# aa217/Neural-Speech-Decoding

Measured on AMD Instinct MI355X. Metric: EEG-trials/sec (train fwd+bwd), higher is better.
Workload: dtype f32; 1 GPU; cfg2: 3-class EEG_LSTM train step (dropout 0.6 + RReLU noise, CE, Adam), 8ch x 250-step windows, H=48 L=2 fp32, batch 256/GPU; batch_per_gpu=256, global_batch=256, T=250, C=8, H=48, L=2, K=3, bidirectional=False, weights=reference checkpoint, parallelism=dp1, launch=eager

## Files before the change

neural-speech-decoding_amd/csrc/nsd_lstm2_bwd48.hip:

```cpp
#include "nsd_args.h"
#include "nsd_multi.h"
#include "nsd_prof.h"
#include "nsd_ring_block.h"
#include "nsd_bf16.h"
#include <type_traits>
#include <utility>

namespace {

constexpr int H = 48;
constexpr int G4 = 192;
constexpr int dl0(const int nb) { return nb == 1 ? 3 : 0; }
constexpr int PRIO1_CHAIN = 2, PRIO1_X1 = 3, PRIO2_CHAIN = 3, PRIO2_X1 = 2, PRIO_LOADER = 1;
constexpr int RING = 8;
constexpr int NTHREADS = 1024;
#ifndef NSD_DW_SLEEP
#define NSD_DW_SLEEP 0
#endif
#ifndef NSD_LD_SLEEP
#define NSD_LD_SLEEP 0
#endif
constexpr int DW_SLEEP = NSD_DW_SLEEP, LD_SLEEP = NSD_LD_SLEEP;
constexpr int CHUNK = 8;
constexpr int REC = 288;
// ... 8 lines not shown
    unsigned short wa[2][2][2][WK][ARS];
    unsigned short wb[2][2][2][WK][BRS];
    float pf[2][2][H][8];
    float din1x[8][H];
};
struct NoWin {};
template <int NB>
struct Smem {
    float ring[2][RING][NB][G4];
    float din1[2][NB][H];
    float stage[2][NB][2][CHUNK][REC];
    float xst[2][NB][CHUNK][8];
    typename std::conditional<NB == 1, DwWin, NoWin>::type win;
};

typedef float f32x2 __attribute__((ext_vector_type(2)));
__device__ __forceinline__ f32x2 pk_fma(f32x2 a, f32x2 b, f32x2 c) { return __builtin_elementwise_fma(a, b, c); }

__device__ __forceinline__ float slice_dot_t(const float *dv, const f32x2 (&wp)[4][6]) {
    f32x2 acc[4];
#pragma unroll
    for (int q = 0; q < 3; ++q) {
        const float4 v = *reinterpret_cast<const float4 *>(dv + 4 * q);
        const f32x2 lo = {v.x, v.y}, hi = {v.z, v.w};
#pragma unroll
        for (int jj = 0; jj < 4; ++jj) {
            acc[jj] = q == 0 ? wp[jj][0] * lo : pk_fma(wp[jj][2 * q], lo, acc[jj]);
            acc[jj] = pk_fma(wp[jj][2 * q + 1], hi, acc[jj]);
        }
    }
    const int lane = threadIdx.x;
    const bool odd = (lane & 1) != 0, hi2 = (lane & 2) != 0;
    const float r0 = acc[0].x + acc[0].y, r1 = acc[1].x + acc[1].y;
    const float r2 = acc[2].x + acc[2].y, r3 = acc[3].x + acc[3].y;
    const float ra = (odd ? r1 : r0) + quad_xor1(odd ? r0 : r1);
    const float rb = (odd ? r3 : r2) + quad_xor1(odd ? r2 : r3);
    float v = (hi2 ? rb : ra) + quad_xor2(hi2 ? ra : rb);
    v += row_ror<4>(v);
    v += row_ror<8>(v);
    return v;
}

__device__ __forceinline__ void load_wT(const float *w, const int og, const int kk, f32x2 (&wp)[4][6]) {
#pragma unroll
    for (int jj = 0; jj < 4; ++jj)
#pragma unroll
        for (int p = 0; p < 6; ++p) {
            wp[jj][p].x = w[(size_t)(12 * kk + 2 * p) * H + 4 * og + jj];
            wp[jj][p].y = w[(size_t)(12 * kk + 2 * p + 1) * H + 4 * og + jj];
        }
}

struct PrepIn { float4 gc; float cprev, ct, mk; float2 ad; };
__device__ __forceinline__ PrepIn prep_load(const Lstm2BwdArgs &a, Smem<1> &sm, const int mn, const int layer, const int u, const float cT1) {
    const int T = a.T;
    const int t = layer == 1 ? T - 1 - mn : T + 1 + dl0(1) - mn;
    const float *rec = &sm.stage[(mn >> 3) & 1][0][layer][mn & 7][0];
    const float *recp = &sm.stage[((mn - 1) >> 3) & 1][0][layer][(mn - 1) & 7][0];
    PrepIn in;
    in.gc = *reinterpret_cast<const float4 *>(rec + 4 * u);
    in.cprev = t > 0 ? rec[192 + u] : 0.f;
    in.ct = t == T - 1 ? cT1 : recp[192 + u];
    in.ad = make_float2(0.f, 0.f); in.mk = 1.f;
    if (layer == 1) in.ad = *reinterpret_cast<const float2 *>(rec + 240);
    else if (a.mask || a.rng.on) in.mk = rec[240 + u];
    return in;
}
__device__ __forceinline__ void prep_finish(Smem<1> &sm, const PrepIn &in, const int mn, const int layer, const int u, const float dpu, const float awu) {
    const float ig = in.gc.x, fg = in.gc.y, gg = in.gc.z, og = in.gc.w;
    const float tc = fast_tanh(in.ct);
    const float x = layer == 1 ? fmaf(in.ad.x, dpu, in.ad.y * awu) : in.mk;
    float *o = &sm.win.pf[mn & 1][layer][u][0];
    *reinterpret_cast<float4 *>(o) = make_float4(og * (1.f - tc * tc), fg, x, 0.f);
    *reinterpret_cast<float4 *>(o + 4) = make_float4(gg * (ig * (1.f - ig)), in.cprev * (fg * (1.f - fg)), ig * (1.f - gg * gg), tc * (og * (1.f - og)));
}
__device__ __forceinline__ void prep_layer(const Lstm2BwdArgs &a, Smem<1> &sm, const int mn, const int layer, const int u,
                                           const float dpu, const float awu, const float cT1) {
    const PrepIn in = prep_load(a, sm, mn, layer, u, cT1);
    prep_finish(sm, in, mn, layer, u, dpu, awu);
}

template <int NB, class A>
__device__ __forceinline__ void chain_role(const A &a, Smem<NB> &sm, const int layer, const int r,
                                           const int n_steps) {
    const int og = r >> 4, kk = r & 15;
    const int j = 4 * og + (r & 3), s = (r >> 2) & 3;
    const int T = a.T, B = a.B;
    const float *cseq = layer == 0 ? a.cseq0 : a.cseq1;
    f32x2 wp[4][6];
    load_wT(layer == 0 ? a.w_hh0 : a.w_hh1, og, kk, wp);
    const float awj = a.attn_w[j];
    float db = 0.f;
    Prof prof = prof_init(a.dbg);

    const int ngrp = (B + NB - 1) / NB;
    for (int grp = wg_id(a); grp < ngrp; grp += wg_count(a)) {
        const int b0 = grp * NB;
        float dc[NB], dhrec[NB], ct[NB], dpj[NB];
#pragma unroll
        for (int n = 0; n < NB; ++n) {
            const int b = b0 + n;
            dc[n] = 0.f; dhrec[n] = 0.f;
            dpj[n] = (NB == 2 && layer == 1 && b < B) ? a.dpooled[(size_t)b * H + j] : 0.f;
            ct[n] = (NB == 2 && b < B) ? cseq[((size_t)b * T + (T - 1)) * H + j] : 0.f;
        }
        step_barrier<false>(prof);

        const int tb = layer == 1 ? T - 1 : T + 1 + dl0(NB);
        for (int m0 = 0; m0 < n_steps; m0 += CHUNK) {
            const int sb = (m0 / CHUNK) & 1;
            ring_block<NB, CHUNK>(m0 >= tb - T + 2 && m0 + CHUNK - 1 <= tb, [&](const int k, const auto inside) {
                const int t = tb - (m0 + k);
                const bool active = inside.value || (t >= 0 && t < T);
                const bool prev_active = inside.value || (t + 1 >= 0 && t + 1 < T);
                if constexpr (NB == 1) {
                    const float *pfl = &sm.win.pf[k & 1][layer][j][0];
                    const float4 pf = *reinterpret_cast<const float4 *>(pfl);
                    const float qr = pfl[4 + s];
                    const float dout = layer == 1 ? pf.z : sm.win.din1x[(k + 6 - dl0(NB)) & 7][j] * pf.z;
                    if (prev_active) dhrec[0] = slice_dot_t(&sm.ring[layer][(k + RING - 1) & (RING - 1)][0][12 * kk], wp);
                    if (active) {
                        const float dht = dout + dhrec[0];
                        const float dct = fmaf(dht, pf.x, dc[0]);
                        const float mine = (s == 3 ? dht : dct) * qr;
                        dc[0] = dct * pf.y;
                        db += mine;
                        sm.ring[layer][k][0][s * H + j] = mine;
                    }
                } else
#pragma unroll
                for (int n = 0; n < NB; ++n) {
                    const float *rec = &sm.stage[sb][n][layer][k][0];
                    const float4 gc = *reinterpret_cast<const float4 *>(rec + 4 * j);
                    const float own = rec[4 * j + s];
                    const float cprev = t > 0 ? rec[192 + j] : 0.f;
                    const float aux0 = layer == 1 ? rec[240] : ((a.mask || a.rng.on) ? rec[240 + j] : 1.f);
                    const float aux1 = rec[241];
                    const float ig = gc.x, fg = gc.y, gg = gc.z, og = gc.w;
                    const float tc = fast_tanh(ct[n]);
                    const float wq = og * (1.f - tc * tc);
                    const float dact = s == 2 ? 1.f - own * own : own * (1.f - own);
                    const float qsel = s == 0 ? gg : s == 1 ? cprev : s == 2 ? ig : tc;
                    const float qr = qsel * dact;
                    float dout;
                    if (layer == 1) dout = fmaf(aux0, dpj[n], aux1 * awj);
                    else            dout = sm.din1[(k + 1) & 1][n][j] * aux0;
                    if (prev_active) dhrec[n] = slice_dot_t(&sm.ring[layer][(k + RING - 1) & (RING - 1)][n][12 * kk], wp);
                    if (active) {
                        float mine = 0.f;
                        if (b0 + n < B) {
                            const float dht = dout + dhrec[n];
                            const float dct = fmaf(dht, wq, dc[n]);
                            mine = (s == 3 ? dht : dct) * qr;
                            dc[n] = dct * fg;
                            db += mine;
                            ct[n] = cprev;
                        }
                        sm.ring[layer][k][n][s * H + j] = mine;
                    }
                }
                step_barrier<false>(prof);
            });
        }
    }
// ... 29 lines not shown
        step_barrier<false>(prof);

        for (int m0 = 0; m0 < n_steps; m0 += CHUNK) {
            const int sb = (m0 / CHUNK) & 1;
#pragma unroll
            for (int k = 0; k < CHUNK; ++k) {
                const int m = m0 + k;
                const int t1p = T - m;
                const int t0p = T + 2 - m;
                constexpr int PREV = RING - 1;
                const int e = (k + PREV) & (RING - 1);
#pragma unroll
                for (int n = 0; n < NB; ++n) {
                    const float2 xv = *reinterpret_cast<const float2 *>(&sm.xst[sb][n][k][2 * s]);
                    if (t1p >= 0 && t1p < T) {
                        float inp = slice_dot_t(&sm.ring[1][e][n][12 * kk], wp);
                        if (a.residual && b0 + n < B) {
                            const float *recp = &sm.stage[k == 0 ? sb ^ 1 : sb][n][1][e][0];
                            inp += fmaf(recp[240], dpj[n], recp[241] * awj);
                        }
                        if (s == 0) sm.din1[k & 1][n][j] = inp;
                    }
                    if (t0p >= 0 && t0p < T && b0 + n < B) {
#pragma unroll
                        for (int g = 0; g < 4; ++g) {
                            const float d = sm.ring[0][e][n][g * H + j];
                            dWih0[g][0] = fmaf(d, xv.x, dWih0[g][0]);
                            dWih0[g][1] = fmaf(d, xv.y, dWih0[g][1]);
                        }
                    }
                }
                step_barrier<false>(prof);
            }
        }
    }
    prof_store(a.dbg, prof);
    float *slab = a.slabs + (size_t)wg_id(a) * a.slab_stride;
#pragma unroll
    for (int g = 0; g < 4; ++g) {
        if (c0 < C) slab[a.o_w_ih0 + (size_t)(g * H + j) * C + c0] = dWih0[g][0];
        if (c1 < C) slab[a.o_w_ih0 + (size_t)(g * H + j) * C + c1] = dWih0[g][1];
    }
}

typedef unsigned u32x2v __attribute__((ext_vector_type(2)));
__device__ __forceinline__ float rows_reduce_scatter4(const f32x4 v) {
    const u32x2v p02 = __builtin_amdgcn_permlane32_swap(__float_as_uint(v[0]), __float_as_uint(v[2]), false, false);
    const u32x2v p13 = __builtin_amdgcn_permlane32_swap(__float_as_uint(v[1]), __float_as_uint(v[3]), false, false);
    const float s02 = __uint_as_float(p02[0]) + __uint_as_float(p02[1]);
    const float s13 = __uint_as_float(p13[0]) + __uint_as_float(p13[1]);
    const u32x2v q = __builtin_amdgcn_permlane16_swap(__float_as_uint(s02), __float_as_uint(s13), false, false);
    return __uint_as_float(q[0]) + __uint_as_float(q[1]);
}
template <class A>
__device__ __forceinline__ void x1m_role(const A &a, Smem<1> &sm, const int g, const int lane, const int n_steps) {
    const int T = a.T, B = a.B;
    const int ks = lane >> 4, ub = (lane >> 2) & 3, jc = lane & 3;
    float wv[H];
#pragma unroll
    for (int sidx = 0; sidx < H; ++sidx) wv[sidx] = a.w_ih1[(size_t)(48 * ks + sidx) * H + 16 * g + 4 * ub + jc];
    const int uo = 16 * g + 4 * ub + ks;
    const float awo = a.attn_w[uo];
    const int pu = lane < H ? lane : lane - 16, pl = g == 0 ? 1 : 0;
    const float p_aw = a.attn_w[pu];
    Prof prof = prof_init(a.dbg);
    for (int grp = wg_id(a); grp < B; grp += wg_count(a)) {
        const int b0 = grp;
        const float dpo = a.residual ? a.dpooled[(size_t)b0 * H + uo] : 0.f;
        float p_dp = 0.f, p_c = 0.f;
        if (g < 2) {
            p_dp = a.dpooled[(size_t)b0 * H + pu];
            p_c = (pl == 1 ? a.cseq1 : a.cseq0)[((size_t)b0 * T + (T - 1)) * H + pu];
        }
#pragma unroll
        for (int s4 = 0; s4 < H; s4 += 8)
            asm volatile("" : "+v"(wv[s4]), "+v"(wv[s4 + 1]), "+v"(wv[s4 + 2]), "+v"(wv[s4 + 3]), "+v"(wv[s4 + 4]), "+v"(wv[s4 + 5]), "+v"(wv[s4 + 6]), "+v"(wv[s4 + 7]));
        step_barrier<false>(prof);
        for (int m0 = 0; m0 < n_steps; m0 += CHUNK) {
#pragma unroll
            for (int k = 0; k < CHUNK; ++k) {
                const int m = m0 + k;
                PrepIn pin;
                if (g < 2) pin = prep_load(a, sm, m + 1, pl, pu, p_c);
                if ((k & 3) == 0 && m >= 4) {
                    const float *vj = &sm.ring[1][(k + 4 + jc) & 7][0][48 * ks];
                    f32x4 acc0 = {0.f, 0.f, 0.f, 0.f}, acc1 = acc0, acc2 = acc0, acc3 = acc0;
#pragma unroll
                    for (int qb = 0; qb < 12; qb += 4) {
                        f32x4 bq[4];
#pragma unroll
                        for (int q = 0; q < 4; ++q) bq[q] = *reinterpret_cast<const f32x4 *>(vj + 4 * (qb + q));
#pragma unroll
                        for (int q = 0; q < 4; ++q) {
                            acc0 = __builtin_amdgcn_mfma_f32_4x4x1f32(wv[4 * (qb + q) + 0], bq[q][0], acc0, 0, 0, 0);
                            acc1 = __builtin_amdgcn_mfma_f32_4x4x1f32(wv[4 * (qb + q) + 1], bq[q][1], acc1, 0, 0, 0);
                            acc2 = __builtin_amdgcn_mfma_f32_4x4x1f32(wv[4 * (qb + q) + 2], bq[q][2], acc2, 0, 0, 0);
                            acc3 = __builtin_amdgcn_mfma_f32_4x4x1f32(wv[4 * (qb + q) + 3], bq[q][3], acc3, 0, 0, 0);
                        }
                    }
                    float inp = rows_reduce_scatter4((acc0 + acc1) + (acc2 + acc3));
                    const int c = m - 4 + jc;
                    if (a.residual) {
                        const float *recp = &sm.stage[(c >> 3) & 1][0][1][c & 7][0];
                        inp += fmaf(recp[240], dpo, recp[241] * awo);
                    }
                    sm.win.din1x[(k + 4 + jc) & 7][uo] = inp;
                }
                if (g < 2) prep_finish(sm, pin, m + 1, pl, pu, p_dp, p_aw);
                if (g == 2 && a.da0_out && m >= 1) {
                    const int t0 = T + 2 + dl0(1) - m;
                    if (t0 >= 0 && t0 < T && lane < H)
                        *reinterpret_cast<f32x4 *>(a.da0_out + ((size_t)b0 * T + t0) * G4 + 4 * lane) =
                            *reinterpret_cast<const f32x4 *>(&sm.ring[0][(k + 7) & 7][0][4 * lane]);
                }
                step_barrier<false>(prof);
            }
        }
    }
    prof_store(a.dbg, prof);
}

template <int NB>
struct DwState {
    f32x4 acc[3][2][3];
    float bq[3][NB][3];
};

template <int Q, int NB>
__device__ __forceinline__ void dw_prefetch(const Lstm2BwdArgs &a, DwState<NB> &st, const int G, const int b0,
                                            const int lane) {
    const int T = a.T, B = a.B;
    const int i = lane & 15, k = lane >> 4;
    const int mm = 4 * G + k;
    const int t = (Q == 2) ? (T + 1 - mm) : (T - 1 - mm);
    const int tt = (Q == 1) ? t : t - 1;
    const bool ok = (t >= 0 && t < T && tt >= 0);
    const float *src = Q == 0 ? a.hseq1 : Q == 1 ? a.in1seq : a.hseq0;
#pragma unroll
    for (int n = 0; n < NB; ++n) {
        const int b = b0 + n;
#pragma unroll
        for (int nt = 0; nt < 3; ++nt)
            st.bq[Q][n][nt] = (ok && b < B) ? src[((size_t)b * T + tt) * H + 16 * nt + i] : 0.f;
    }
}

template <int Q, int NB>
__device__ __forceinline__ void dw_compute(const Lstm2BwdArgs &a, Smem<NB> &sm, DwState<NB> &st, const int G,
                                           const int dwid, const int lane) {
    const int T = a.T;
    const int i = lane & 15, k = lane >> 4;
    const int mm = 4 * G + k;
    constexpr int layer = (Q == 2) ? 0 : 1;
    const int t = layer == 1 ? (T - 1 - mm) : (T + 1 - mm);
    const bool ok = (t >= 0 && t < T);
#pragma unroll
    for (int n = 0; n < NB; ++n) {
        float av[2];
#pragma unroll
        for (int mt = 0; mt < 2; ++mt) {
            const float v = sm.ring[layer][mm & (RING - 1)][n][32 * dwid + 16 * mt + i];
            av[mt] = ok ? v : 0.f;
        }
#pragma unroll
        for (int mt = 0; mt < 2; ++mt)
#pragma unroll
            for (int nt = 0; nt < 3; ++nt)
                st.acc[Q][mt][nt] = __builtin_amdgcn_mfma_f32_16x16x4f32(av[mt], st.bq[Q][n][nt], st.acc[Q][mt][nt], 0, 0, 0);
    }
}

template <class A>
// ... 34 lines not shown
            dw_prefetch<1, NB>(a, st, G, b0, lane);
            step_barrier<false, DW_SLEEP>(prof);
            if (G > 0 && !ablated(a.ablate, 1)) dw_compute<2, NB>(a, sm, st, G - 1, dwid, lane);
            dw_prefetch<2, NB>(a, st, G, b0, lane);
            step_barrier<false, DW_SLEEP>(prof);
            step_barrier<false, DW_SLEEP>(prof);
        }
        if (!ablated(a.ablate, 1)) {
            dw_compute<0, NB>(a, sm, st, n_groups - 1, dwid, lane);
            dw_compute<1, NB>(a, sm, st, n_groups - 1, dwid, lane);
            dw_compute<2, NB>(a, sm, st, n_groups - 1, dwid, lane);
        }
    }
    prof_store(a.dbg, prof);
    float *slab = a.slabs + (size_t)wg_id(a) * a.slab_stride;
    const long base[3] = {a.o_w_hh1, a.o_w_ih1, a.o_w_hh0};
#pragma unroll
    for (int q = 0; q < 3; ++q)
#pragma unroll
        for (int mt = 0; mt < 2; ++mt)
#pragma unroll
            for (int nt = 0; nt < 3; ++nt)
#pragma unroll
                for (int rr = 0; rr < 4; ++rr) {
                    const int row = 32 * dwid + 16 * mt + 4 * (lane >> 4) + rr;
                    const int col = 16 * nt + (lane & 15);
                    slab[base[q] + (size_t)row * H + col] = st.acc[q][mt][nt][rr];
                }
}

template <class F, int... I>
__device__ __forceinline__ void static_for(F &&f, std::integer_sequence<int, I...>) { (f(std::integral_constant<int, I>{}), ...); }
__device__ __forceinline__ void split1_bf16(const float v, unsigned short &hi, unsigned short &lo) {
    const unsigned h = pack_bf16x2(v, 0.f);
    hi = (unsigned short)h;
    lo = (unsigned short)pack_bf16x2(v - bf16_lo(h), 0.f);
}
template <int RS>
__device__ __forceinline__ bf16x8 window_frag(const unsigned short *win, const int c0, const int lane) {
    const int G = lane >> 4, i = lane & 15;
    const unsigned short *p = win + (8 * (G >> 1) + (i >> 2)) * RS + c0 + 16 * (G & 1) + 4 * (i & 3);
    const s16x4 e0 = lds_read_tr16(reinterpret_cast<const bf16_t *>(p));
    const s16x4 e1 = lds_read_tr16(reinterpret_cast<const bf16_t *>(p + 4 * RS));
    return cat_tr(e0, e1);
}

__device__ __forceinline__ void split4_bf16(const f32x4 v, u32x2 &hi, u32x2 &lo) {
    hi[0] = pack_bf16x2(v[0], v[1]);
    hi[1] = pack_bf16x2(v[2], v[3]);
    lo[0] = pack_bf16x2(v[0] - bf16_lo(hi[0]), v[1] - bf16_hi(hi[0]));
    lo[1] = pack_bf16x2(v[2] - bf16_lo(hi[1]), v[3] - bf16_hi(hi[1]));
}

template <class A>
__device__ __forceinline__ void dw16_role(const A &a_in, Smem<1> &sm, const int w_in, const int lane, const int n_steps_in) {
    const int w = __builtin_amdgcn_readfirstlane(w_in), n_steps = __builtin_amdgcn_readfirstlane(n_steps_in);
    const A a = uniform_copy(a_in);
    DwWin &win = sm.win;
    const int T = a.T, B = a.B, C = a.C;
    Prof prof = prof_init(a.dbg);
    f32x16 acc[5];
#pragma unroll
    for (int q = 0; q < 5; ++q) acc[q] = zero16();
    const int l48 = lane < 48 ? lane : lane - 16;
    const float *src = w == 0 ? a.hseq1 : w == 1 ? a.in1seq : w == 2 ? a.hseq0 : a.x;
    const int rw = w == 3 ? C : H;
    const int rs = w == 3 ? lane >> 4 : l48 / 12, rp = w == 3 ? lane & 15 : l48 - 12 * rs;
    const int rl = w < 2 ? 1 : 0;
    const int rc = w == 3 ? H + rp : (w == 1 ? H : 0) + 4 * rp;
    const long sbytes = (long)B * T * rw * 4;
    const __amdgpu_buffer_rsrc_t r_s = __builtin_amdgcn_make_buffer_rsrc(const_cast<float *>(src), 0, (int)(sbytes > 0x7fffffffL ? 0x7fffffffL : sbytes), 0x00020000);
    constexpr unsigned DROP = 0x80000000u;
    const int L = w * 64 + lane, mk_k = L / H, mk_j = L - mk_k * H;
    auto gen_mask = [&](const int chunk, const int b) {
        const int t = T + 1 + dl0(1) - (chunk * CHUNK + mk_k);
        if (t >= 0 && t < T)
            sm.stage[chunk & 1][0][0][mk_k][240 + mk_j] =
                nsd_rand_u32(a.rng.seed, a.rng.base, ((uint64_t)b * T + t) * H + mk_j) < a.rng.thr_lstm ? 0.f : a.rng.keep_lstm;
    };
    bf16x8 ah, al;
    auto a_frags = [&](const int W, const int layer) {
        ah = window_frag<ARS>(&win.wa[layer][0][W & 1][0][0], 32 * w, lane);
        al = window_frag<ARS>(&win.wa[layer][1][W & 1][0][0], 32 * w, lane);
    };
    auto tile = [&](const int W, auto qc) {
        constexpr int q = decltype(qc)::value;
        constexpr int layer = q < 3 ? 1 : 0, ni = q < 3 ? q : q - 3;
        if (q == 0 || q == 3) a_frags(W, layer);
        const bf16x8 bh = window_frag<BRS>(&win.wb[layer][0][W & 1][0][0], 32 * ni, lane);
        const bf16x8 bl = window_frag<BRS>(&win.wb[layer][1][W & 1][0][0], 32 * ni, lane);
        if (!ablated(a.ablate, 1)) {
            acc[q] = __builtin_amdgcn_mfma_f32_32x32x16_bf16(ah, bh, acc[q], 0, 0, 0);
            acc[q] = __builtin_amdgcn_mfma_f32_32x32x16_bf16(al, bh, acc[q], 0, 0, 0);
            acc[q] = __builtin_amdgcn_mfma_f32_32x32x16_bf16(ah, bl, acc[q], 0, 0, 0);
        }
    };
    {
        u32x4 *z = reinterpret_cast<u32x4 *>(&win.wb[0][0][0][0][0]);
        constexpr int NZ = (int)(sizeof(win.wb) / 16);
        const u32x4 zero = {0u, 0u, 0u, 0u};
        for (int e = w * 64 + lane; e < NZ; e += 6 * 64) z[e] = zero;
    }
    const int ngrp = B;
    for (int grp = wg_id(a); grp < ngrp; grp += wg_count(a)) {
        const int b = grp;
        if (a.rng.on) gen_mask(0, b);
        auto request = [&](const int m) -> f32x4 {
            const int t = (rl == 1 ? T - 1 : T + 1 + dl0(1)) - m - rs;
            const int tt = (w == 1 || w == 3) ? t : t - 1;
            const bool ok = t >= 0 && t < T && tt >= 0 && (w != 3 || rp < C);
            f32x4 v = {0.f, 0.f, 0.f, 0.f};
            if (w == 3) {
                const unsigned off = ok ? (unsigned)((((size_t)b * T + tt) * C + rp) * 4) : DROP;
                v[0] = __uint_as_float(__builtin_amdgcn_raw_buffer_load_b32(r_s, (int)off, 0, 0));
            } else {
                const unsigned off = ok ? (unsigned)((((size_t)b * T + tt) * H + 4 * rp) * 4) : DROP;
                v = __builtin_bit_cast(f32x4, __builtin_amdgcn_raw_buffer_load_b128(r_s, (int)off, 0, 0));
            }
            return v;
        };
        f32x4 bq = {0.f, 0.f, 0.f, 0.f};
        if (w < 4) bq = request(0);
        step_barrier<false>(prof);
        auto half = [&](const int m0, auto phc) {
            constexpr int PH = decltype(phc)::value;
            static_for([&](auto kc) {
                constexpr int k = decltype(kc)::value;
                const int m = m0 + k;
                constexpr int p = PH + k;
                const int wi = (m >> 4) & 1;
                if (w >= 4 && m >= 1) {
                    const int mm = m - 1, cl = 5 - w;
                    const int t = cl == 1 ? T - 1 - mm : T + 1 + dl0(1) - mm;
                    f32x4 v = *reinterpret_cast<const f32x4 *>(&sm.ring[cl][mm & (RING - 1)][0][4 * l48]);
                    if (!(t >= 0 && t < T)) v = f32x4{0.f, 0.f, 0.f, 0.f};
                    u32x2 hi, lo;
                    split4_bf16(v, hi, lo);
                    *reinterpret_cast<u32x2 *>(&win.wa[cl][0][(mm >> 4) & 1][mm & 15][4 * l48]) = hi;
                    *reinterpret_cast<u32x2 *>(&win.wa[cl][1][(mm >> 4) & 1][mm & 15][4 * l48]) = lo;
                }
                if (w < 4 && (k & 3) == 0) {
                    if (w == 3) {
                        unsigned short hi, lo;
                        split1_bf16(bq[0], hi, lo);
                        win.wb[0][0][wi][p + rs][rc] = hi;
                        win.wb[0][1][wi][p + rs][rc] = lo;
                    } else {
                        u32x2 hi, lo;
                        split4_bf16(bq, hi, lo);
                        *reinterpret_cast<u32x2 *>(&win.wb[rl][0][wi][p + rs][rc]) = hi;
                        *reinterpret_cast<u32x2 *>(&win.wb[rl][1][wi][p + rs][rc]) = lo;
                    }
                    __builtin_amdgcn_sched_barrier(0);
                    bq = request(m + 4);
                }
                if (a.rng.on && k == 1) gen_mask((m >> 3) + 1, b);
                if (p >= 1 && p <= 5 && m >= 17) tile((m - 17) >> 4, std::integral_constant<int, (p >= 1 && p <= 5) ? p - 1 : 0>{});
                step_barrier<false, DW_SLEEP>(prof);
            }, std::make_integer_sequence<int, 8>{});
        };
        for (int m0 = 0; m0 < n_steps; m0 += 16) {
            half(m0, std::integral_constant<int, 0>{});
            if (m0 + 8 < n_steps) half(m0 + 8, std::integral_constant<int, 8>{});
        }
        {
            const int Wl = (n_steps - 1) >> 4, cl = lane >> 5, cc = 32 * w + (lane & 31);
            const int k0 = (n_steps - 1) & 15;
            for (int k = k0; k < 16; ++k) {
                win.wa[cl][0][Wl & 1][k][cc] = 0;
                win.wa[cl][1][Wl & 1][k][cc] = 0;
            }
            tile(Wl, std::integral_constant<int, 0>{});
            tile(Wl, std::integral_constant<int, 1>{});
            tile(Wl, std::integral_constant<int, 2>{});
            tile(Wl, std::integral_constant<int, 3>{});
            tile(Wl, std::integral_constant<int, 4>{});
        }
    }
    prof_store(a.dbg, prof);
    float *slab = a.slabs + (size_t)wg_id(a) * a.slab_stride;
#pragma unroll
    for (int q = 0; q < 5; ++q) {
        const int layer = q < 3 ? 1 : 0, c = 32 * (q < 3 ? q : q - 3) + (lane & 31);
        const long base = layer == 1 ? (c < H ? a.o_w_hh1 : a.o_w_ih1) : (c < H ? a.o_w_hh0 : a.o_w_ih0);
        const int ld = (layer == 0 && c >= H) ? C : H, col = c < H ? c : c - H;
        const bool okc = layer == 1 || c < H + C;
#pragma unroll
        for (int r = 0; r < 16; ++r) {
            const int row = 32 * w + mfma32_row(r, lane);
            if (okc) slab[base + (size_t)row * ld + col] = acc[q][r];
        }
    }
}

constexpr int NQ = STAGE_F4 / 64;

struct LdDesc {
    const char *base;
    int row_bytes;
    int t0;
};

template <int NB>
__device__ __forceinline__ void loader_decode(const Lstm2BwdArgs &a, const int lane, LdDesc (&d)[NQ]) {
    const int T = a.T;
#pragma unroll
    for (int q = 0; q < NQ; ++q) {
        const int e = q * 64 + lane;
        const int layer = e / (CHUNK * REC4);
        const int rem = e - layer * (CHUNK * REC4);
        const int k = rem / REC4, w = rem - k * REC4;
        d[q].t0 = layer == 1 ? (T - 1 - k) : (T + 1 + dl0(NB) - k);
        d[q].row_bytes = 0;
        d[q].base = nullptr;
        if (w < 48) {
            d[q].base = (const char *)((layer == 0 ? a.gact0 : a.gact1) + w * 4); d[q].row_bytes = H * 16;
        } else if (w < 60) {
            d[q].base = (const char *)((layer == 0 ? a.cseq0 : a.cseq1) + (w - 48) * 4) - H * 4; d[q].row_bytes = H * 4;
        } else if (layer == 0) {
            if (a.mask && !a.rng.on) { d[q].base = (const char *)(a.mask + (w - 60) * 4); d[q].row_bytes = H * 4; }
        } else if (w == 60) {
            d[q].base = (const char *)a.dsc_pack; d[q].row_bytes = 16;
        }
    }
}

template <int NB, int Q0, int Q1>
__device__ __forceinline__ void loader_issue(const Lstm2BwdArgs &a, Smem<NB> &sm, const LdDesc (&d)[NQ], const int chunk,
                                             const int buf, const int b0) {
    const int T = a.T;
#pragma unroll
    for (int n = 0; n < NB; ++n) {
        const int b = b0 + n;
        if (b < a.B) {
#pragma unroll
            for (int q = Q0; q < Q1; ++q) {
                const int t = d[q].t0 - CHUNK * chunk;
                if (d[q].row_bytes != 0 && (unsigned)t < (unsigned)T) {
                    const char *src = d[q].base + (size_t)((unsigned)(b * T + t)) * (unsigned)d[q].row_bytes;
                    __builtin_amdgcn_global_load_lds((const void *)src,
                                                     (__attribute__((address_space(3))) void *)(&sm.stage[buf][n][0][0][0] + q * 256),
                                                     16, 0, 0);
                }
            }
        }
// ... 34 lines not shown
        loader_issue<NB, 0, NQ>(a, sm, d, 0, 0, b0);
        if (NB == 2) loader_issue_x<NB>(a, sm, 0, 0, b0, lane);
        asm volatile("s_waitcnt vmcnt(0)" ::: "memory");
        if constexpr (NB == 1) { prep_layer(a, sm, 0, 1, u, dpu, awu, cT1[1]); prep_layer(a, sm, 0, 0, u, dpu, awu, cT1[0]); }
        step_barrier<true>(prof);
        for (int m0 = 0; m0 < n_steps; m0 += CHUNK) {
            const int chunk = m0 / CHUNK, nb = (chunk + 1) & 1;
            const bool on = !ablated(a.ablate, 16);
            if constexpr (NB == 1) {
                if (on) loader_issue<NB, 0, 4>(a, sm, d, chunk + 1, nb, b0);
                step_barrier<true, LD_SLEEP>(prof);
                if (on) loader_issue<NB, 4, 8>(a, sm, d, chunk + 1, nb, b0);
                step_barrier<true, LD_SLEEP>(prof);
                if (on) loader_issue<NB, 8, 12>(a, sm, d, chunk + 1, nb, b0);
                step_barrier<true, LD_SLEEP>(prof);
                if (on) loader_issue<NB, 12, 16>(a, sm, d, chunk + 1, nb, b0);
                step_barrier<true, LD_SLEEP>(prof);
                if (on) loader_issue<NB, 16, 18>(a, sm, d, chunk + 1, nb, b0);
                step_barrier<true, LD_SLEEP>(prof);
                step_barrier<true, LD_SLEEP>(prof);
                asm volatile("s_waitcnt vmcnt(0)" ::: "memory");
                step_barrier<true, LD_SLEEP>(prof);
                step_barrier<true, LD_SLEEP>(prof);
            } else {
            if (on) { loader_issue<NB, 0, 3>(a, sm, d, chunk + 1, nb, b0); if (NB == 2) loader_issue_x<NB>(a, sm, chunk + 1, nb, b0, lane); }
            step_barrier<true, LD_SLEEP>(prof);
            if (on) loader_issue<NB, 3, 6>(a, sm, d, chunk + 1, nb, b0);
            step_barrier<true, LD_SLEEP>(prof);
            if (on) loader_issue<NB, 6, 9>(a, sm, d, chunk + 1, nb, b0);
            step_barrier<true, LD_SLEEP>(prof);
            if (on) loader_issue<NB, 9, 12>(a, sm, d, chunk + 1, nb, b0);
            step_barrier<true, LD_SLEEP>(prof);
            if (on) loader_issue<NB, 12, 15>(a, sm, d, chunk + 1, nb, b0);
            step_barrier<true, LD_SLEEP>(prof);
            if (on) loader_issue<NB, 15, 18>(a, sm, d, chunk + 1, nb, b0);
            step_barrier<true, LD_SLEEP>(prof);
            step_barrier<true, LD_SLEEP>(prof);
            asm volatile("s_waitcnt vmcnt(0)" ::: "memory");
            step_barrier<true, LD_SLEEP>(prof);
            }
        }
    }
    prof_store(a.dbg, prof);
}

#define NSD_B48_ROLE_TABLE(VIEW) \
    if constexpr (NB == 1) { \
        constexpr int ROLE[16] = {0, 0, 0, 1, 1, 1, 2, 2, 2, 3, 3, 3, 3, 3, 3, 4}; \
        constexpr int PART[16] = {0, 1, 2, 0, 1, 2, 0, 1, 2, 4, 2, 3, 0, 1, 5, 0}; \
        const int lane = tid & 63; \
        const int role = ROLE[wave], part = PART[wave]; \
        if (role == 0)      { VIEW; __builtin_amdgcn_s_setprio(PRIO1_CHAIN); chain_role<NB>(a, sm, 1, 64 * part + lane, n_steps); } \
        else if (role == 1) { VIEW; __builtin_amdgcn_s_setprio(PRIO1_CHAIN); chain_role<NB>(a, sm, 0, 64 * part + lane, n_steps); } \
        else if (role == 2) { VIEW; __builtin_amdgcn_s_setprio(PRIO1_X1); x1m_role(a, sm, part, lane, n_steps); } \
        else if (role == 3) { VIEW; dw16_role(a, sm, part, lane, n_steps); } \
        else                { VIEW; __builtin_amdgcn_s_setprio(PRIO_LOADER); loader_role<NB>(a, sm, lane, n_steps); } \
    } else { \
        if (wave < 3)       { VIEW; __builtin_amdgcn_s_setprio(PRIO2_CHAIN); chain_role<NB>(a, sm, 1, tid, n_steps); } \
        else if (wave < 6)  { VIEW; __builtin_amdgcn_s_setprio(PRIO2_CHAIN); chain_role<NB>(a, sm, 0, tid - 192, n_steps); } \
        else if (wave < 9)  { VIEW; __builtin_amdgcn_s_setprio(PRIO2_X1); x1_role(a, sm, tid - 384, n_steps); } \
        else if (wave < 15) { VIEW; dw_role(a, sm, wave - 9, tid & 63, n_groups); } \
        else                { VIEW; __builtin_amdgcn_s_setprio(PRIO_LOADER); loader_role<NB>(a, sm, tid & 63, n_steps); } \
    }

#if !NSD_MULTI_TU
template <int NB>
__global__ __launch_bounds__(NTHREADS) void lstm2_bwd48_kernel(Lstm2BwdArgs a) {
    __shared__ __align__(16) Smem<NB> sm;
    const int tid = threadIdx.x;
    const int wave = __builtin_amdgcn_readfirstlane(tid >> 6);
    const int n_groups = (((a.T + 2 + dl0(NB)) / 4 + 1) + 1) & ~1;
    const int n_steps = 4 * n_groups;
    NSD_B48_ROLE_TABLE()
}

#else
template <int NB>
__global__ __launch_bounds__(NTHREADS) void lstm2_bwd48_multi_kernel(Lstm2BwdArgs a_in, ModelSplit s) {
    __shared__ __align__(16) Smem<NB> sm;
    const int tid = threadIdx.x;
    const int wave = __builtin_amdgcn_readfirstlane(tid >> 6);
    const int n_groups = (((a_in.T + 2 + dl0(NB)) / 4 + 1) + 1) & ~1;
    const int n_steps = 4 * n_groups;
    NSD_B48_ROLE_TABLE(const ModelView<Lstm2BwdArgs> a = model_view(a_in, s))
}

#endif
#undef NSD_B48_ROLE_TABLE

}

static int bwd48_domain(const Lstm2BwdArgs &a, int nb, bool models, const char *who) {
    if (nb == 1 && (long)a.B * a.T * H * 4 >= 0x7fffffffL) nb = 2;
    if (a.da0_out && models) { nsd_set_error("%s: no input gradient on the model-batched path", who); return 0; }
    if (a.da0_out && nb != 1) { nsd_set_error("%s: the input gradient needs the one-trial instantiation (B * T * H * 4 < 2 GB)", who); return 0; }
    if (nb != 1 && nb != 2) { nsd_set_error("%s: NB=%d not built (register / LDS budget)", who, nb); return 0; }
    return nb;
}

#if !NSD_MULTI_TU
int nsd_lstm2_bwd48_launch(const Lstm2BwdArgs &a, int nb, int grid, hipStream_t st) {
    nb = bwd48_domain(a, nb, false, "lstm2_bwd48");
    if (nb == 0) return NSD_E_INVALID;
    if (nb == 1) hipLaunchKernelGGL((lstm2_bwd48_kernel<1>), dim3(grid), dim3(NTHREADS), 0, st, a);
    else         hipLaunchKernelGGL((lstm2_bwd48_kernel<2>), dim3(grid), dim3(NTHREADS), 0, st, a);
    NSD_CHECK_LAUNCH("lstm2_bwd48");
    return NSD_OK;
}
// ... 12 lines not shown
```

neural-speech-decoding_amd/csrc/nsd_ring_block.h:

```cpp
#pragma once
#include <hip/hip_runtime.h>
#include <type_traits>

template <int NB, int N, class Body>
__device__ __forceinline__ void ring_block(const bool inside, Body &&body) {
    if constexpr (NB == 1) {
        if (inside) {
#pragma unroll
            for (int k = 0; k < N; ++k) body(k, std::true_type{});
        } else {
#pragma unroll 1
            for (int k = 0; k < N; ++k) body(k, std::false_type{});
        }
    } else {
#pragma unroll
        for (int k = 0; k < N; ++k) body(k, std::false_type{});
    }
}
```

Baseline: 1.100 million trials/s.

## Specialize x1m and dw16 roles on duty/flags and drop boundary checks inside

The x1m and dw16 wave roles become templates on their duty index and runtime flags (residual, dx output, RNG), with dispatchers, so per-step branches on those flags become compile-time. Interior chunks take an 'inside' path that drops time-boundary checks, using shared schedule predicates moved into a header. dw16 also precomputes LDS base pointers in address space 3 and uses direct transposed LDS reads plus 32-bit offset math. This is meant to cut scalar/vector overhead in the hot per-step loops, at the cost of more code instantiations and instruction-cache pressure.

```diff
diff --git a/neural-speech-decoding_amd/csrc/nsd_lstm2_bwd48.hip b/neural-speech-decoding_amd/csrc/nsd_lstm2_bwd48.hip
--- a/neural-speech-decoding_amd/csrc/nsd_lstm2_bwd48.hip
+++ b/neural-speech-decoding_amd/csrc/nsd_lstm2_bwd48.hip
@@ -84,18 +84,18 @@
 }
 
 struct PrepIn { float4 gc; float cprev, ct, mk; float2 ad; };
-__device__ __forceinline__ PrepIn prep_load(const Lstm2BwdArgs &a, Smem<1> &sm, const int mn, const int layer, const int u, const float cT1) {
-    const int T = a.T;
+template <bool INSIDE = false>
+__device__ __forceinline__ PrepIn prep_load(const int T, const bool has_mk, Smem<1> &sm, const int mn, const int layer, const int u, const float cT1) {
     const int t = layer == 1 ? T - 1 - mn : T + 1 + dl0(1) - mn;
     const float *rec = &sm.stage[(mn >> 3) & 1][0][layer][mn & 7][0];
     const float *recp = &sm.stage[((mn - 1) >> 3) & 1][0][layer][(mn - 1) & 7][0];
     PrepIn in;
     in.gc = *reinterpret_cast<const float4 *>(rec + 4 * u);
-    in.cprev = t > 0 ? rec[192 + u] : 0.f;
-    in.ct = t == T - 1 ? cT1 : recp[192 + u];
+    in.cprev = (INSIDE || t > 0) ? rec[192 + u] : 0.f;
+    in.ct = (!INSIDE && t == T - 1) ? cT1 : recp[192 + u];
     in.ad = make_float2(0.f, 0.f); in.mk = 1.f;
     if (layer == 1) in.ad = *reinterpret_cast<const float2 *>(rec + 240);
-    else if (a.mask || a.rng.on) in.mk = rec[240 + u];
+    else if (has_mk) in.mk = rec[240 + u];
     return in;
 }
 __device__ __forceinline__ void prep_finish(Smem<1> &sm, const PrepIn &in, const int mn, const int layer, const int u, const float dpu, const float awu) {
@@ -108,7 +108,7 @@
 }
 __device__ __forceinline__ void prep_layer(const Lstm2BwdArgs &a, Smem<1> &sm, const int mn, const int layer, const int u,
                                            const float dpu, const float awu, const float cT1) {
-    const PrepIn in = prep_load(a, sm, mn, layer, u, cT1);
+    const PrepIn in = prep_load(a.T, a.mask || a.rng.on, sm, mn, layer, u, cT1);
     prep_finish(sm, in, mn, layer, u, dpu, awu);
 }
 
@@ -141,7 +141,7 @@
         const int tb = layer == 1 ? T - 1 : T + 1 + dl0(NB);
         for (int m0 = 0; m0 < n_steps; m0 += CHUNK) {
             const int sb = (m0 / CHUNK) & 1;
-            ring_block<NB, CHUNK>(m0 >= tb - T + 2 && m0 + CHUNK - 1 <= tb, [&](const int k, const auto inside) {
+            ring_block<NB, CHUNK>(h48_bwd_sched::chain_inside(layer, T, m0, dl0(NB)), [&](const int k, const auto inside) {
                 const int t = tb - (m0 + k);
                 const bool active = inside.value || (t >= 0 && t < T);
                 const bool prev_active = inside.value || (t + 1 >= 0 && t + 1 < T);
@@ -277,8 +277,13 @@
     const u32x2v q = __builtin_amdgcn_permlane16_swap(__float_as_uint(s02), __float_as_uint(s13), false, false);
     return __uint_as_float(q[0]) + __uint_as_float(q[1]);
 }
-template <class A>
-__device__ __forceinline__ void x1m_role(const A &a, Smem<1> &sm, const int g, const int lane, const int n_steps) {
+template <int DUTY, bool RES, bool DX, class A>
+__device__ __forceinline__ void x1m_role(const A &a, Smem<1> &sm, const int lane_in, const int n_steps) {
+    static_assert(!DX || DUTY < 0, "the input gradient's operand leaves from the wave without a prep duty");
+    int lane = lane_in;
+    asm volatile("; x1m %1" : "+v"(lane) : "n"(4 * (DUTY + 1) + 2 * (RES ? 1 : 0) + (DX ? 1 : 0)));
+    constexpr int g = DUTY == 1 ? 0 : DUTY == 0 ? 1 : 2;
+    constexpr int sched = DUTY == 1 ? h48_bwd_sched::X1_PREP1 : DUTY == 0 ? h48_bwd_sched::X1_PREP0 : DX ? h48_bwd_sched::X1_DX : h48_bwd_sched::X1_PLAIN;
     const int T = a.T, B = a.B;
     const int ks = lane >> 4, ub = (lane >> 2) & 3, jc = lane & 3;
     float wv[H];
@@ -286,14 +291,16 @@
     for (int sidx = 0; sidx < H; ++sidx) wv[sidx] = a.w_ih1[(size_t)(48 * ks + sidx) * H + 16 * g + 4 * ub + jc];
     const int uo = 16 * g + 4 * ub + ks;
     const float awo = a.attn_w[uo];
-    const int pu = lane < H ? lane : lane - 16, pl = g == 0 ? 1 : 0;
+    constexpr int pl = DUTY == 1 ? 1 : 0;
+    const int pu = lane < H ? lane : lane - 16;
     const float p_aw = a.attn_w[pu];
+    const bool has_mk = a.mask || a.rng.on;
     Prof prof = prof_init(a.dbg);
     for (int grp = wg_id(a); grp < B; grp += wg_count(a)) {
         const int b0 = grp;
-        const float dpo = a.residual ? a.dpooled[(size_t)b0 * H + uo] : 0.f;
+        const float dpo = RES ? a.dpooled[(size_t)b0 * H + uo] : 0.f;
         float p_dp = 0.f, p_c = 0.f;
-        if (g < 2) {
+        if constexpr (DUTY >= 0) {
             p_dp = a.dpooled[(size_t)b0 * H + pu];
             p_c = (pl == 1 ? a.cseq1 : a.cseq0)[((size_t)b0 * T + (T - 1)) * H + pu];
         }
@@ -302,12 +309,12 @@
             asm volatile("" : "+v"(wv[s4]), "+v"(wv[s4 + 1]), "+v"(wv[s4 + 2]), "+v"(wv[s4 + 3]), "+v"(wv[s4 + 4]), "+v"(wv[s4 + 5]), "+v"(wv[s4 + 6]), "+v"(wv[s4 + 7]));
         step_barrier<false>(prof);
         for (int m0 = 0; m0 < n_steps; m0 += CHUNK) {
-#pragma unroll
-            for (int k = 0; k < CHUNK; ++k) {
+            ring_block<1, CHUNK>(h48_bwd_sched::x1m_inside(sched, T, m0), [&](const int k, const auto inside) {
+                constexpr bool IN = decltype(inside)::value;
                 const int m = m0 + k;
                 PrepIn pin;
-                if (g < 2) pin = prep_load(a, sm, m + 1, pl, pu, p_c);
-                if ((k & 3) == 0 && m >= 4) {
+                if constexpr (DUTY >= 0) pin = prep_load<IN>(T, has_mk, sm, m + 1, pl, pu, p_c);
+                if ((k & 3) == 0 && (IN || m >= 4)) {
                     const float *vj = &sm.ring[1][(k + 4 + jc) & 7][0][48 * ks];
                     f32x4 acc0 = {0.f, 0.f, 0.f, 0.f}, acc1 = acc0, acc2 = acc0, acc3 = acc0;
 #pragma unroll
@@ -325,24 +332,36 @@
                     }
                     float inp = rows_reduce_scatter4((acc0 + acc1) + (acc2 + acc3));
                     const int c = m - 4 + jc;
-                    if (a.residual) {
+                    if constexpr (RES) {
                         const float *recp = &sm.stage[(c >> 3) & 1][0][1][c & 7][0];
                         inp += fmaf(recp[240], dpo, recp[241] * awo);
                     }
                     sm.win.din1x[(k + 4 + jc) & 7][uo] = inp;
                 }
-                if (g < 2) prep_finish(sm, pin, m + 1, pl, pu, p_dp, p_aw);
-                if (g == 2 && a.da0_out && m >= 1) {
+                if constexpr (DUTY >= 0) prep_finish(sm, pin, m + 1, pl, pu, p_dp, p_aw);
+                if constexpr (DX) {
                     const int t0 = T + 2 + dl0(1) - m;
-                    if (t0 >= 0 && t0 < T && lane < H)
+                    if ((IN || (m >= 1 && t0 >= 0 && t0 < T)) && lane < H)
                         *reinterpret_cast<f32x4 *>(a.da0_out + ((size_t)b0 * T + t0) * G4 + 4 * lane) =
                             *reinterpret_cast<const f32x4 *>(&sm.ring[0][(k + 7) & 7][0][4 * lane]);
                 }
                 step_barrier<false>(prof);
-            }
+            });
         }
     }
     prof_store(a.dbg, prof);
+}
+template <class A>
+__device__ __forceinline__ void x1m_dispatch(const A &a, Smem<1> &sm, const int part, const int lane, const int n_steps) {
+    if (part == 0) {
+        if (a.residual) x1m_role<1, true, false>(a, sm, lane, n_steps); else x1m_role<1, false, false>(a, sm, lane, n_steps);
+    } else if (part == 1) {
+        if (a.residual) x1m_role<0, true, false>(a, sm, lane, n_steps); else x1m_role<0, false, false>(a, sm, lane, n_steps);
+    } else if (a.da0_out) {
+        if (a.residual) x1m_role<-1, true, true>(a, sm, lane, n_steps); else x1m_role<-1, false, true>(a, sm, lane, n_steps);
+    } else {
+        if (a.residual) x1m_role<-1, true, false>(a, sm, lane, n_steps); else x1m_role<-1, false, false>(a, sm, lane, n_steps);
+    }
 }
 
 template <int NB>
@@ -483,9 +502,23 @@
     lo[1] = pack_bf16x2(v[2] - bf16_lo(hi[1]), v[3] - bf16_hi(hi[1]));
 }
 
-template <class A>
-__device__ __forceinline__ void dw16_role(const A &a_in, Smem<1> &sm, const int w_in, const int lane, const int n_steps_in) {
-    const int w = __builtin_amdgcn_readfirstlane(w_in), n_steps = __builtin_amdgcn_readfirstlane(n_steps_in);
+#define NSD_LDS __attribute__((address_space(3)))
+typedef NSD_LDS unsigned short lds_u16;
+constexpr int SA_W = WK * ARS, SA_HL = 2 * SA_W, SA_L = 2 * SA_HL;
+constexpr int SB_W = WK * BRS, SB_HL = 2 * SB_W, SB_L = 2 * SB_HL;
+static_assert(sizeof(DwWin::wa) < 65536 && sizeof(DwWin::wb) < 65536, "a window region within reach of one lane base");
+template <int RS>
+__device__ __forceinline__ bf16x8 lds_frag(const lds_u16 *p) {
+    const s16x4 e0 = __builtin_amdgcn_ds_read_tr16_b64_v4i16((s16x4 NSD_LDS *)(p));
+    const s16x4 e1 = __builtin_amdgcn_ds_read_tr16_b64_v4i16((s16x4 NSD_LDS *)(p + 4 * RS));
+    return cat_tr(e0, e1);
+}
+template <int DUTY, bool RNG, class A>
+__device__ __forceinline__ void dw16_role(const A &a_in, Smem<1> &sm, const int lane_in, const int n_steps_in) {
+    constexpr int w = DUTY;
+    int lane = lane_in;
+    asm volatile("; dw16 %1" : "+v"(lane) : "n"(2 * DUTY + (RNG ? 1 : 0)));
+    const int n_steps = __builtin_amdgcn_readfirstlane(n_steps_in);
     const A a = uniform_copy(a_in);
     DwWin &win = sm.win;
     const int T = a.T, B = a.B, C = a.C;
@@ -497,29 +530,48 @@
     const float *src = w == 0 ? a.hseq1 : w == 1 ? a.in1seq : w == 2 ? a.hseq0 : a.x;
     const int rw = w == 3 ? C : H;
     const int rs = w == 3 ? lane >> 4 : l48 / 12, rp = w == 3 ? lane & 15 : l48 - 12 * rs;
-    const int rl = w < 2 ? 1 : 0;
+    constexpr int rl = w < 2 ? 1 : 0;
     const int rc = w == 3 ? H + rp : (w == 1 ? H : 0) + 4 * rp;
     const long sbytes = (long)B * T * rw * 4;
     const __amdgpu_buffer_rsrc_t r_s = __builtin_amdgcn_make_buffer_rsrc(const_cast<float *>(src), 0, (int)(sbytes > 0x7fffffffL ? 0x7fffffffL : sbytes), 0x00020000);
     constexpr unsigned DROP = 0x80000000u;
-    const int L = w * 64 + lane, mk_k = L / H, mk_j = L - mk_k * H;
+    constexpr int cl = w >= 4 ? 5 - w : 0;
+    lds_u16 *fa, *fb, *cw = nullptr, *rwp = nullptr;
+    const NSD_LDS float *cr = nullptr;
+    {
+        const int G = lane >> 4, i = lane & 15;
+        fa = (lds_u16 *)(&win.wa[0][0][0][0][0]) + (8 * (G >> 1) + (i >> 2)) * ARS + 32 * w + 16 * (G & 1) + 4 * (i & 3);
+        fb = (lds_u16 *)(&win.wb[0][0][0][0][0]) + (8 * (G >> 1) + (i >> 2)) * BRS + 16 * (G & 1) + 4 * (i & 3);
+        if constexpr (w >= 4) {
+            cw = (lds_u16 *)(&win.wa[cl][0][0][0][0]) + 4 * l48;
+            cr = (const NSD_LDS float *)(&sm.ring[cl][0][0][0]) + 4 * l48;
+        } else {
+            rwp = (lds_u16 *)(&win.wb[rl][0][0][0][0]) + rs * BRS + rc;
+        }
+    }
+    int mk_k = 0, mk_c = 0, mk_o = 0;
+    if constexpr (RNG) {
+        const int L = w * 64 + lane, mk_j = L - (L / H) * H;
+        mk_k = L / H; mk_c = mk_j - mk_k * H; mk_o = mk_k * REC + 240 + mk_j;
+    }
     auto gen_mask = [&](const int chunk, const int b) {
-        const int t = T + 1 + dl0(1) - (chunk * CHUNK + mk_k);
+        asm volatile("" : "+v"(mk_k), "+v"(mk_c), "+v"(mk_o));
+        const int tc = T + 1 + dl0(1) - chunk * CHUNK, t = tc - mk_k;
         if (t >= 0 && t < T)
-            sm.stage[chunk & 1][0][0][mk_k][240 + mk_j] =
-                nsd_rand_u32(a.rng.seed, a.rng.base, ((uint64_t)b * T + t) * H + mk_j) < a.rng.thr_lstm ? 0.f : a.rng.keep_lstm;
+            (&sm.stage[chunk & 1][0][0][0][0])[mk_o] =
+                nsd_rand_u32(a.rng.seed, a.rng.base, ((uint64_t)b * T + tc) * H + (int64_t)mk_c) < a.rng.thr_lstm ? 0.f : a.rng.keep_lstm;
     };
     bf16x8 ah, al;
-    auto a_frags = [&](const int W, const int layer) {
-        ah = window_frag<ARS>(&win.wa[layer][0][W & 1][0][0], 32 * w, lane);
-        al = window_frag<ARS>(&win.wa[layer][1][W & 1][0][0], 32 * w, lane);
-    };
-    auto tile = [&](const int W, auto qc) {
+    auto tile = [&](const int Wn, auto qc) {
         constexpr int q = decltype(qc)::value;
         constexpr int layer = q < 3 ? 1 : 0, ni = q < 3 ? q : q - 3;
-        if (q == 0 || q == 3) a_frags(W, layer);
-        const bf16x8 bh = window_frag<BRS>(&win.wb[layer][0][W & 1][0][0], 32 * ni, lane);
-        const bf16x8 bl = window_frag<BRS>(&win.wb[layer][1][W & 1][0][0], 32 * ni, lane);
+        const lds_u16 *faw = fa + (Wn & 1) * SA_W, *fbw = fb + (Wn & 1) * SB_W;
+        if (q == 0 || q == 3) {
+            ah = lds_frag<ARS>(faw + layer * SA_L);
+            al = lds_frag<ARS>(faw + layer * SA_L + SA_HL);
+        }
+        const bf16x8 bh = lds_frag<BRS>(fbw + layer * SB_L + 32 * ni);
+        const bf16x8 bl = lds_frag<BRS>(fbw + layer * SB_L + SB_HL + 32 * ni);
         if (!ablated(a.ablate, 1)) {
             acc[q] = __builtin_amdgcn_mfma_f32_32x32x16_bf16(ah, bh, acc[q], 0, 0, 0);
             acc[q] = __builtin_amdgcn_mfma_f32_32x32x16_bf16(al, bh, acc[q], 0, 0, 0);
@@ -535,17 +587,17 @@
     const int ngrp = B;
     for (int grp = wg_id(a); grp < ngrp; grp += wg_count(a)) {
         const int b = grp;
-        if (a.rng.on) gen_mask(0, b);
+        if (RNG) gen_mask(0, b);
         auto request = [&](const int m) -> f32x4 {
             const int t = (rl == 1 ? T - 1 : T + 1 + dl0(1)) - m - rs;
             const int tt = (w == 1 || w == 3) ? t : t - 1;
             const bool ok = t >= 0 && t < T && tt >= 0 && (w != 3 || rp < C);
             f32x4 v = {0.f, 0.f, 0.f, 0.f};
             if (w == 3) {
-                const unsigned off = ok ? (unsigned)((((size_t)b * T + tt) * C + rp) * 4) : DROP;
+                const unsigned off = ok ? ((unsigned)(b * T + tt) * (unsigned)C + (unsigned)rp) * 4u : DROP;
                 v[0] = __uint_as_float(__builtin_amdgcn_raw_buffer_load_b32(r_s, (int)off, 0, 0));
             } else {
-                const unsigned off = ok ? (unsigned)((((size_t)b * T + tt) * H + 4 * rp) * 4) : DROP;
+                const unsigned off = ok ? ((unsigned)(b * T + tt) * (unsigned)H + 4u * (unsigned)rp) * 4u : DROP;
                 v = __builtin_bit_cast(f32x4, __builtin_amdgcn_raw_buffer_load_b128(r_s, (int)off, 0, 0));
             }
             return v;
@@ -553,53 +605,78 @@
         f32x4 bq = {0.f, 0.f, 0.f, 0.f};
         if (w < 4) bq = request(0);
         step_barrier<false>(prof);
-        auto half = [&](const int m0, auto phc) {
+        auto half = [&](const int m0, auto phc, auto firstc, auto insidec) {
             constexpr int PH = decltype(phc)::value;
+            constexpr bool FIRST = decltype(firstc)::value, INSIDE = decltype(insidec)::value;
+            asm volatile("" : "+v"(fa), "+v"(fb));
+            if constexpr (w >= 4) asm volatile("" : "+v"(cw), "+v"(cr)); else asm volatile("" : "+v"(rwp));
+            const int wi = (m0 >> 4) & 1;
             static_for([&](auto kc) {
                 constexpr int k = decltype(kc)::value;
                 const int m = m0 + k;
                 constexpr int p = PH + k;
-                const int wi = (m >> 4) & 1;
-                if (w >= 4 && m >= 1) {
-                    const int mm = m - 1, cl = 5 - w;
+                if constexpr (w >= 4) if (INSIDE || m >= 1) {
+                    const int mm = m - 1;
+                    constexpr int pm = (p + 15) & 15;
+                    const int wm = p == 0 ? wi ^ 1 : wi;
                     const int t = cl == 1 ? T - 1 - mm : T + 1 + dl0(1) - mm;
-                    f32x4 v = *reinterpret_cast<const f32x4 *>(&sm.ring[cl][mm & (RING - 1)][0][4 * l48]);
-                    if (!(t >= 0 && t < T)) v = f32x4{0.f, 0.f, 0.f, 0.f};
+                    f32x4 v = *reinterpret_cast<const NSD_LDS f32x4 *>(cr + ((k + RING - 1) & (RING - 1)) * G4);
+                    if (!INSIDE && !(t >= 0 && t < T)) v = f32x4{0.f, 0.f, 0.f, 0.f};
                     u32x2 hi, lo;
                     split4_bf16(v, hi, lo);
-                    *reinterpret_cast<u32x2 *>(&win.wa[cl][0][(mm >> 4) & 1][mm & 15][4 * l48]) = hi;
-                    *reinterpret_cast<u32x2 *>(&win.wa[cl][1][(mm >> 4) & 1][mm & 15][4 * l48]) = lo;
+                    *reinterpret_cast<NSD_LDS u32x2 *>(cw + wm * SA_W + pm * ARS) = hi;
+                    *reinterpret_cast<NSD_LDS u32x2 *>(cw + wm * SA_W + pm * ARS + SA_HL) = lo;
                 }
-                if (w < 4 && (k & 3) == 0) {
+                if constexpr (w < 4 && (k & 3) == 0) {
                     if (w == 3) {
                         unsigned short hi, lo;
                         split1_bf16(bq[0], hi, lo);
-                        win.wb[0][0][wi][p + rs][rc] = hi;
-                        win.wb[0][1][wi][p + rs][rc] = lo;
+                        rwp[wi * SB_W + p * BRS] = hi;
+                        rwp[wi * SB_W + p * BRS + SB_HL] = lo;
                     } else {
                         u32x2 hi, lo;
                         split4_bf16(bq, hi, lo);
-                        *reinterpret_cast<u32x2 *>(&win.wb[rl][0][wi][p + rs][rc]) = hi;
-                        *reinterpret_cast<u32x2 *>(&win.wb[rl][1][wi][p + rs][rc]) = lo;
+                        *reinterpret_cast<NSD_LDS u32x2 *>(rwp + wi * SB_W + p * BRS) = hi;
+                        *reinterpret_cast<NSD_LDS u32x2 *>(rwp + wi * SB_W + p * BRS + SB_HL) = lo;
                     }
                     __builtin_amdgcn_sched_barrier(0);
                     bq = request(m + 4);
                 }
-                if (a.rng.on && k == 1) gen_mask((m >> 3) + 1, b);
-                if (p >= 1 && p <= 5 && m >= 17) tile((m - 17) >> 4, std::integral_constant<int, (p >= 1 && p <= 5) ? p - 1 : 0>{});
+                if (RNG && k == 1) gen_mask((m >> 3) + 1, b);
+                if (p >= 1 && p <= 5 && !FIRST) tile((m - 17) >> 4, std::integral_constant<int, (p >= 1 && p <= 5) ? p - 1 : 0>{});
                 step_barrier<false, DW_SLEEP>(prof);
             }, std::make_integer_sequence<int, 8>{});
         };
-        for (int m0 = 0; m0 < n_steps; m0 += 16) {
-            half(m0, std::integral_constant<int, 0>{});
-            if (m0 + 8 < n_steps) half(m0 + 8, std::integral_constant<int, 8>{});
-        }
+        constexpr auto PH0 = std::integral_constant<int, 0>{};
+        constexpr auto PH8 = std::integral_constant<int, 8>{};
+        auto second_half = [&](const int m0) {
+            bool in = true;
+            if constexpr (DUTY >= 4) in = h48_bwd_sched::dw_conv_inside(5 - DUTY, T, m0);
+            if (in) half(m0, PH8, std::false_type{}, std::true_type{});
+            else    half(m0, PH8, std::false_type{}, std::false_type{});
+        };
+        int m0 = 0;
+        asm volatile("" : "+s"(m0));
+        half(m0, PH0, std::true_type{}, std::integral_constant<bool, (DUTY < 4)>{});
+        if (8 < n_steps) second_half(m0 + 8);
+        m0 += 16;
+        for (; m0 < n_steps && (DUTY < 4 || h48_bwd_sched::dw_conv_inside(5 - DUTY, T, m0)); m0 += 16) {
+            half(m0, PH0, std::false_type{}, std::true_type{});
+            if (m0 + 8 < n_steps) second_half(m0 + 8);
+        }
+        if constexpr (DUTY >= 4)
+            for (; m0 < n_steps; m0 += 16) {
+                half(m0, PH0, std::false_type{}, std::false_type{});
+                if (m0 + 8 < n_steps) second_half(m0 + 8);
+            }
         {
-            const int Wl = (n_steps - 1) >> 4, cl = lane >> 5, cc = 32 * w + (lane & 31);
+            int lz = lane;
+            asm volatile("" : "+v"(lz), "+v"(fa), "+v"(fb));
+            const int Wl = (n_steps - 1) >> 4, zl = lz >> 5, cc = 32 * w + (lz & 31);
             const int k0 = (n_steps - 1) & 15;
             for (int k = k0; k < 16; ++k) {
-                win.wa[cl][0][Wl & 1][k][cc] = 0;
-                win.wa[cl][1][Wl & 1][k][cc] = 0;
+                win.wa[zl][0][Wl & 1][k][cc] = 0;
+                win.wa[zl][1][Wl & 1][k][cc] = 0;
             }
             tile(Wl, std::integral_constant<int, 0>{});
             tile(Wl, std::integral_constant<int, 1>{});
@@ -622,6 +699,16 @@
             if (okc) slab[base + (size_t)row * ld + col] = acc[q][r];
         }
     }
+}
+#undef NSD_LDS
+template <class A>
+__device__ __forceinline__ void dw16_dispatch(const A &a, Smem<1> &sm, const int part, const int lane, const int n_steps) {
+    static_for([&](auto wc) {
+        constexpr int W = decltype(wc)::value;
+        if (part == W) {
+            if (a.rng.on) dw16_role<W, true>(a, sm, lane, n_steps); else dw16_role<W, false>(a, sm, lane, n_steps);
+        }
+    }, std::make_integer_sequence<int, 6>{});
 }
 
 constexpr int NQ = STAGE_F4 / 64;
@@ -762,8 +849,8 @@
         const int role = ROLE[wave], part = PART[wave]; \
         if (role == 0)      { VIEW; __builtin_amdgcn_s_setprio(PRIO1_CHAIN); chain_role<NB>(a, sm, 1, 64 * part + lane, n_steps); } \
         else if (role == 1) { VIEW; __builtin_amdgcn_s_setprio(PRIO1_CHAIN); chain_role<NB>(a, sm, 0, 64 * part + lane, n_steps); } \
-        else if (role == 2) { VIEW; __builtin_amdgcn_s_setprio(PRIO1_X1); x1m_role(a, sm, part, lane, n_steps); } \
-        else if (role == 3) { VIEW; dw16_role(a, sm, part, lane, n_steps); } \
+        else if (role == 2) { VIEW; __builtin_amdgcn_s_setprio(PRIO1_X1); x1m_dispatch(a, sm, part, lane, n_steps); } \
+        else if (role == 3) { VIEW; dw16_dispatch(a, sm, part, lane, n_steps); } \
         else                { VIEW; __builtin_amdgcn_s_setprio(PRIO_LOADER); loader_role<NB>(a, sm, lane, n_steps); } \
     } else { \
         if (wave < 3)       { VIEW; __builtin_amdgcn_s_setprio(PRIO2_CHAIN); chain_role<NB>(a, sm, 1, tid, n_steps); } \
diff --git a/neural-speech-decoding_amd/csrc/nsd_ring_block.h b/neural-speech-decoding_amd/csrc/nsd_ring_block.h
--- a/neural-speech-decoding_amd/csrc/nsd_ring_block.h
+++ b/neural-speech-decoding_amd/csrc/nsd_ring_block.h
@@ -1,6 +1,39 @@
 #pragma once
+#ifdef __HIPCC__
 #include <hip/hip_runtime.h>
+#endif
 #include <type_traits>
+
+#ifndef __HIPCC__
+#define NSD_SCHED_FN constexpr
+#else
+#define NSD_SCHED_FN __host__ __device__ constexpr
+#endif
+namespace h48_bwd_sched {
+constexpr int BLOCK = 8;
+constexpr int DL0 = 3;
+NSD_SCHED_FN int n_steps(const int T, const int dl0 = DL0) { return 4 * ((((T + 2 + dl0) / 4 + 1) + 1) & ~1); }
+NSD_SCHED_FN int tbase(const int layer, const int T, const int dl0 = DL0) { return layer == 1 ? T - 1 : T + 1 + dl0; }
+NSD_SCHED_FN bool chain_inside(const int layer, const int T, const int m0, const int dl0 = DL0) {
+    return m0 >= tbase(layer, T, dl0) - T + 2 && m0 + BLOCK - 1 <= tbase(layer, T, dl0);
+}
+enum X1Duty : int { X1_PREP1 = 0, X1_PREP0 = 1, X1_PLAIN = 2, X1_DX = 3 };
+NSD_SCHED_FN bool x1m_inside(const int duty, const int T, const int m0) {
+    if (m0 < BLOCK) return false;
+    const int mlast = m0 + BLOCK - 1;
+    if (duty == X1_PREP1) return tbase(1, T) - (mlast + 1) > 0;
+    if (duty == X1_PREP0) return tbase(0, T) - (mlast + 1) > 0;
+    if (duty == X1_DX) return T + 2 + DL0 - mlast >= 0;
+    return true;
+}
+NSD_SCHED_FN bool dw_conv_inside(const int layer, const int T, const int m0) {
+    return m0 >= BLOCK && tbase(layer, T) - (m0 - 1) < T && tbase(layer, T) - (m0 + BLOCK - 2) >= 0;
+}
+NSD_SCHED_FN bool dw_tiles(const int m0) { return m0 >= 2 * BLOCK; }
+}
+#undef NSD_SCHED_FN
+
+#ifdef __HIPCC__
 
 template <int NB, int N, class Body>
 __device__ __forceinline__ void ring_block(const bool inside, Body &&body) {
@@ -17,3 +50,4 @@
         for (int k = 0; k < N; ++k) body(k, std::false_type{});
     }
 }
+#endif
```

Measured after the change: 1.143 million trials/s (median of 6 runs). +3.8%, better.
